# Brown-LEMS/Edge_Based_Visual_Odometry

Hardware: AMD Instinct MI355X
Metric: stereo pairs/sec (TOED+NCC match) on KITTI 1241×376; achieved HBM GB/s (higher is better)
Workload: dtype f64; 1 GPU; configs[1]: single KITTI-shaped stereo pair 1241x376 (generator S2, scene 7+rank, 12 px disparity), TOED both images (fp64, no FMA, bit-exact) + epipolar/disparity/orientation candidate search + NCC, resident in HBM, replayed; toed_mode=hybrid, edges_left=126184, edges_right=126340, candidate_pairs=581657, ncc_matches=472947, sims_stored=False, pairs_in_flight_per_gpu=6, streams_per_gpu=4, pairs_submitted_as_hipgraph=2331, toed_strict_fallbacks=0, parallelism=1 independent sequence(s), one per GPU, no collective

## Files before the change

### edge_based_visual_odometry_amd/csrc/toed_kernels.hip

```cpp
#include <cstring>

#include <hip/hip_ext.h>

#include "ebvo_internal.h"
#include <atomic>
#include "ebvo_math.h"

namespace
{

const double h_TAP_INT[4][19] = {
    {7.99187055345274e-06, 6.69151128824427e-05, 0.000436341347522880, 0.00221592420596900,
     0.00876415024678427, 0.0269954832565940, 0.0647587978329459, 0.120985362259572, 0.176032663382150,
     0.199471140200716, 0.176032663382150, 0.120985362259572, 0.0647587978329459, 0.0269954832565940,
     0.00876415024678427, 0.00221592420596900, 0.000436341347522880, 6.69151128824427e-05,
     7.99187055345274e-06},
    {1.79817087452687e-05, 0.000133830225764885, 0.000763597358165040, 0.00332388630895351,
     0.0109551878084803, 0.0269954832565940, 0.0485690983747094, 0.0604926811297858, 0.0440081658455374, 0,
     -0.0440081658455374, -0.0604926811297858, -0.0485690983747094, -0.0269954832565940,
     -0.0109551878084803, -0.00332388630895351, -0.000763597358165040, -0.000133830225764885,
     -1.79817087452687e-05},
    {3.84608770384913e-05, 0.000250931673309160, 0.00122721003990810, 0.00443184841193801,
     0.0115029471989044, 0.0202466124424455, 0.0202371243227956, 0, -0.0330061243841531,
     -0.0498677850501791, -0.0330061243841531, 0, 0.0202371243227956, 0.0202466124424455,
// ... 569 lines not shown
        {
            const v2f ti0 = *reinterpret_cast<const v2f *>(L.tap[0][0]), ti18 = *reinterpret_cast<const v2f *>(L.tap[0][18]);
            const v2f th0 = *reinterpret_cast<const v2f *>(L.tap[1][0]), th18 = *reinterpret_cast<const v2f *>(L.tap[1][18]);
#pragma unroll
            for (int c = 0; c < 4; ++c)
            {
                const float xl = v[c + HALO + 9], xr = v[c + HALO - 9];
                const v2f l2 = (v2f){xl, xl}, r2 = (v2f){xr, xr};
                const v2f i19 = __builtin_elementwise_fma(r2, ti18, __builtin_elementwise_fma(l2, ti0, a17[c]));
                const v2f h19 = __builtin_elementwise_fma(r2, th18, __builtin_elementwise_fma(l2, th0, ah[c]));
                o[0][c] = a17[c].x;
                o[1][c] = a17[c].y;
                o[2][c] = i19.x;
                o[3][c] = i19.y;
                o[4][c] = h19.x;
                o[5][c] = h19.y;
            }
        }
#pragma unroll
        for (int k = 0; k < 6; ++k)
            *reinterpret_cast<float4 *>(&L.R[k][r][c0]) = make_float4(o[k][0], o[k][1], o[k][2], o[k][3]);
    }
    __syncthreads();
    const int c = tid & 31, ph = (tid >> 5) & 3, sy = ph >> 1, sx = ph & 1, e0 = (tid >> 7) * 7;
    float fx[7], fy[7], mg[7];
    {
        const int base = sx ? 4 : (sy ? 2 : 0);
        const int pm = (ph == 0) ? 8 : 9;
        v2f rr[25];
#pragma unroll
        for (int k = 0; k < 25; ++k)
            rr[k] = (v2f){L.R[base + 1][e0 + k][c], L.R[base][e0 + k][c]};
        v2f acc[7];
#pragma unroll
        for (int e = 0; e < 7; ++e)
            acc[e] = (v2f){0.0f, 0.0f};
#pragma unroll
        for (int p = -9; p <= 9; ++p)
        {
            if (p < -pm || p > pm)
                continue;
            const v2f kk = *reinterpret_cast<const v2f *>(L.tap[sy][p + 9]);
#pragma unroll
            for (int e = 0; e < 7; ++e)
                acc[e] = __builtin_elementwise_fma(rr[e + HALO - p], kk, acc[e]);
        }
#pragma unroll
        for (int e = 0; e < 7; ++e)
        {
            fx[e] = acc[e].x;
            fy[e] = acc[e].y;
        }
        const float dcx = T->screen_dc[ph][0], dcy = T->screen_dc[ph][1];
#pragma unroll
        for (int e = 0; e < 7; ++e)
        {
            fx[e] += dcx;
            fy[e] += dcy;
            mg[e] = __builtin_sqrtf(__builtin_fmaf(fx[e], fx[e], fy[e] * fy[e]));
        }
    }
    __syncthreads();
#pragma unroll
    for (int e = 0; e < 7; ++e)
        L.M[ph][e0 + e][c] = mg[e];
    __syncthreads();
    const float *Mflat = &L.M[0][0][0];
    auto row_step = [&](int da) { return ((((sy + da) & 1) - sy) * 2 * FE_H + ((sy + da) >> 1)) * FE_W; };
    auto col_step = [&](int db) { return (((sx + db) & 1) - sx) * FE_H * FE_W + ((sx + db) >> 1); };
    const int rdn = row_step(-1), rup = row_step(1), cdn = col_step(-1), cup = col_step(1);
    const int lane = tid & 63;
#pragma unroll
    for (int e = 0; e < 7; ++e)
    {
        const int er = e0 + e;
        const int i = i0 + er, j = j0 + c;
        const int I = 2 * i + sy, J = 2 * j + sx;
        int f = 0;
        const bool mine = er >= 1 && er <= FT_H && c >= 1 && c <= FT_W && I >= 10 && I < H2 - 10 && J >= 10 && J < W2 - 10;
        if (mine)
        {
            const float m = mg[e];
            if (m > 2.0f - SCREEN_TOL_M)
            {
                const float gx = fx[e], gy = fy[e], ax = fabsf(gx), ay = fabsf(gy);
                if (ax < SCREEN_TOL_M || ay < SCREEN_TOL_M || fabsf(ax - ay) < SCREEN_TOL_M)
                {
                    const bool px = gx >= 0, py = gy >= 0;
                    const int ctr = (ph * FE_H + er) * FE_W + c;
                    const int rP = py ? rup : rdn, rM = py ? rdn : rup, cP = px ? cup : cdn, cM = px ? cdn : cup;
                    float np, nm, dp, dm, w_up;
                    if (ay < SCREEN_TOL_M || ax < SCREEN_TOL_M)
                    {
                        const bool xd = ay < SCREEN_TOL_M;
                        const int aP = xd ? cP : rP, aM = xd ? cM : rM, o1 = xd ? rup : cup, o2 = xd ? rdn : cdn;
                        np = Mflat[ctr + aP];
                        nm = Mflat[ctr + aM];
                        dp = fmaxf(fabsf(Mflat[ctr + aP + o1] - np), fabsf(Mflat[ctr + aP + o2] - np));
                        dm = fmaxf(fabsf(Mflat[ctr + aM + o1] - nm), fabsf(Mflat[ctr + aM + o2] - nm));
                        w_up = 2.0f * SCREEN_TOL_M / (xd ? ax : ay);
                    }
                    else
                    {
                        np = Mflat[ctr + rP + cP];
                        nm = Mflat[ctr + rM + cM];
                        dp = fmaxf(fabsf(Mflat[ctr + cP] - np), fabsf(Mflat[ctr + rP] - np));
                        dm = fmaxf(fabsf(Mflat[ctr + cM] - nm), fabsf(Mflat[ctr + rM] - nm));
                        w_up = 2.0f * SCREEN_TOL_M / fmaxf(ax, ay);
                    }
                    if (m >= np - (SCREEN_TOL_M + w_up * dp) && m >= nm - (SCREEN_TOL_M + w_up * dm))
                        f = 1;
                }
                else
                {
                    const bool px = gx >= 0, py = gy >= 0;
                    const bool xdom = px ? (py ? gx >= gy : !(gx < ay)) : (py ? !(ax < gy) : ax >= ay);
                    const float num = xdom ? ((px == py) ? gy : -gy) : ((px == py) ? gx : -gx);
                    const float den = xdom ? gx : gy;
                    const float slope = num / den;
                    const int ctr = (ph * FE_H + er) * FE_W + c;
                    const int rP = py ? rup : rdn, rM = py ? rdn : rup, cP = px ? cup : cdn, cM = px ? cdn : cup;
                    const float p1 = Mflat[ctr + (xdom ? cP : rP)], p2 = Mflat[ctr + rP + cP];
                    const float m1 = Mflat[ctr + (xdom ? cM : rM)], m2 = Mflat[ctr + rM + cM];
                    const float fp = p1 * (1 - slope) + p2 * slope;
                    const float fm = m1 * (1 - slope) + m2 * slope;
                    const float tp = SCREEN_TOL_M + SCREEN_TOL_S * fabsf(p2 - p1);
                    const float tm = SCREEN_TOL_M + SCREEN_TOL_S * fabsf(m2 - m1);
                    if (m >= fm - tm && m >= fp - tp)
                        f = 1;
                }
            }
            B.flag[blockIdx.z][(size_t)I * W2 + J] = (uint8_t)f;
            if (DIAG)
            {
                float *dp = D.plane[blockIdx.z];
                const size_t plane = (size_t)H2 * W2, o = (size_t)I * W2 + J;
                dp[o] = fx[e];
                dp[plane + o] = fy[e];
                dp[2 * plane + o] = mg[e];
            }
        }
        const unsigned long long any = __ballot(f != 0);
        if (lane == 0 && any)
        {
            const int ne = __popcll(any & 0xffffffffull), no = __popcll(any >> 32);
            if (ne)
                atomicAdd(&B.row_cnt[blockIdx.z][I], ne);
            if (no)
                atomicAdd(&B.row_cnt[blockIdx.z][H2 + I], no);
        }
    }
}

__global__ __launch_bounds__(256) void toed_compact_phase_kernel(ImgBatch B, int h, int w, int cap)
{
    const int W2 = 2 * w, H2 = 2 * h;
    const int i = 10 + blockIdx.x;
    if (i >= H2 - 10)
        return;
    const uint8_t *flag = B.flag[blockIdx.y] + (size_t)i * W2;
    const int32_t *cnt = B.row_cnt[blockIdx.y];
    int32_t *src = B.src[blockIdx.y];
    int32_t *lists = B.lists[blockIdx.y];
    __shared__ int w_all[4], w_par[2][4], s_sum[4][4];
    const int lane = threadIdx.x & 63, wid = threadIdx.x >> 6;
    auto sum_rows = [&](int r_end, int out[4]) {
        int a[4] = {0, 0, 0, 0};
        for (int r = threadIdx.x; r < r_end; r += 256)
        {
            a[(r & 1) * 2 + 0] += cnt[r];
            a[(r & 1) * 2 + 1] += cnt[H2 + r];
        }
#pragma unroll
        for (int k = 0; k < 4; ++k)
            for (int d = 32; d > 0; d >>= 1)
                a[k] += __shfl_down(a[k], d);
        __syncthreads();
        if (lane == 0)
#pragma unroll
            for (int k = 0; k < 4; ++k)
                s_sum[wid][k] = a[k];
        __syncthreads();
#pragma unroll
        for (int k = 0; k < 4; ++k)
            out[k] = s_sum[0][k] + s_sum[1][k] + s_sum[2][k] + s_sum[3][k];
    };
    int pre[4];
    sum_rows(i, pre);
    if (blockIdx.x == 0)
    {
        int tot[4];
        sum_rows(H2, tot);
        if (threadIdx.x == 0)
        {
            const int all = tot[0] + tot[1] + tot[2] + tot[3];
            const bool over = all > cap;
            int32_t *counts = B.counts[blockIdx.y], *lcount = B.lcount[blockIdx.y];
            counts[2] = over ? 0 : all;
            counts[3] = 0;
            counts[4] = all;
            for (int ph = 0; ph < 4; ++ph)
                lcount[ph] = over ? 0 : tot[ph];
            for (int k = 4; k < 12; ++k)
                lcount[k] = 0;
        }
    }
    int base_all = pre[0] + pre[1] + pre[2] + pre[3];
    int base_ph[2] = {pre[(i & 1) * 2], pre[(i & 1) * 2 + 1]};
    const int par = threadIdx.x & 1;
    const unsigned long long pmask = par ? 0xaaaaaaaaaaaaaaaaull : 0x5555555555555555ull;
    for (int j0 = 10; j0 < W2 - 10; j0 += 256)
    {
        const int j = j0 + threadIdx.x;
        const int f = (j < W2 - 10) ? flag[j] : 0;
        const unsigned long long m_all = __ballot(f != 0);
        const unsigned long long below = (1ull << lane) - 1ull;
        if (lane == 0)
        {
            w_all[wid] = __popcll(m_all);
            w_par[0][wid] = __popcll(m_all & 0x5555555555555555ull);
            w_par[1][wid] = __popcll(m_all & 0xaaaaaaaaaaaaaaaaull);
        }
        __syncthreads();
        int pre_all = 0, tot_all = 0, pre_ph = 0, tot_ph[2] = {0, 0};
#pragma unroll
        for (int k = 0; k < 4; ++k)
        {
            if (k < wid)
            {
                pre_all += w_all[k];
                pre_ph += w_par[par][k];
            }
            tot_all += w_all[k];
            tot_ph[0] += w_par[0][k];
            tot_ph[1] += w_par[1][k];
        }
        if (f)
        {
            const int r_all = base_all + pre_all + __popcll(m_all & below);
            if (r_all < cap)
            {
                src[2 * r_all] = i * W2 + j;
                src[2 * r_all + 1] = -1;
                const int ph = ((i & 1) << 1) | par;
                lists[(size_t)ph * cap + base_ph[par] + pre_ph + __popcll(m_all & pmask & below)] = r_all;
            }
        }
        base_all += tot_all;
        base_ph[0] += tot_ph[0];
        base_ph[1] += tot_ph[1];
        __syncthreads();
    }
}

struct __attribute__((aligned(64))) CandExact
{
    double gx, gy, m, tox, toy;
    int32_t sector;
    int32_t pad0;
    double pad1[2];
};
static_assert(sizeof(CandExact) == 64, "one cache line per candidate");

__host__ __device__ inline size_t mag_tiles_per_row(int W2) { return (size_t)((W2 + 3) >> 2); }
__host__ __device__ inline size_t mag_map_doubles(int H2, int W2) { return (size_t)((H2 + 1) >> 1) * mag_tiles_per_row(W2) * 8; }
__host__ __device__ inline size_t mag_index(int I, int J, int W2)
{
    return ((size_t)(I >> 1) * mag_tiles_per_row(W2) + (size_t)(J >> 2)) * 8 + (size_t)(((I & 1) << 2) | (J & 3));
}

struct ExactBatch
{
    const uint8_t *img[MAX_BATCH];
    const int32_t *src[MAX_BATCH];
    const int32_t *counts[MAX_BATCH];
    int32_t *lists[MAX_BATCH];
    int32_t *lcount[MAX_BATCH];
    CandExact *cd[MAX_BATCH];
    CandRec *rec[MAX_BATCH];
    int32_t *cand_flag[MAX_BATCH];
    int2 *chunk_cnt[MAX_BATCH];
    const uint8_t *flag[MAX_BATCH];
    uint32_t *needbits[MAX_BATCH];
    int32_t *need_cnt[MAX_BATCH];
    double *magmap[MAX_BATCH];
};

__device__ inline void block_append(bool put, int value, int32_t *__restrict__ list, int32_t *__restrict__ counter,
                                    int *s_cnt )
{
    const int lane = threadIdx.x & 63, wid = threadIdx.x >> 6;
    const unsigned long long m = __ballot(put);
    if (lane == 0)
        s_cnt[wid] = __popcll(m);
    __syncthreads();
    if (threadIdx.x == 0)
    {
        const int tot = s_cnt[0] + s_cnt[1] + s_cnt[2] + s_cnt[3];
        s_cnt[4] = tot ? atomicAdd(counter, tot) : 0;
    }
    __syncthreads();
    if (put)
    {
        int pre = 0;
        for (int k = 0; k < wid; ++k)
            pre += s_cnt[k];
        list[s_cnt[4] + pre + __popcll(m & ((1ull << lane) - 1ull))] = value;
    }
    __syncthreads();
}

struct Row24
{
    unsigned long long w0, w1, w2;
};

__device__ inline Row24 fetch_row(const uint8_t *__restrict__ img, int h, int w, int ii, int j)
{
    const int ic = min(max(ii, 0), h - 1);
    const uint8_t *p = img + (size_t)ic * w + (j - HALO);
    Row24 r;
    __builtin_memcpy(&r.w0, p, 8);
    __builtin_memcpy(&r.w1, p + 8, 8);
    __builtin_memcpy(&r.w2, p + 16, 8);
    return r;
}

struct ColMask
{
    unsigned m[5];
};
__device__ inline ColMask column_mask(int w, int j)
{
    const int lo = max(0, HALO - j), hi = min(19, w + HALO - j);
    ColMask c;
#pragma unroll
    for (int d = 0; d < 5; ++d)
    {
        const int a = min(max(lo - 4 * d, 0), 4), b = min(max(hi - 4 * d, 0), 4);
        const unsigned upto_b = b >= 4 ? 0xffffffffu : ((1u << (8 * b)) - 1u);
        const unsigned upto_a = a >= 4 ? 0xffffffffu : ((1u << (8 * a)) - 1u);
        c.m[d] = upto_b & ~upto_a;
    }
    return c;
}

__device__ inline void unpack_row(const Row24 &r, int h, int ii, const ColMask &cm, bool fast, int v[19])
{
    unsigned d[5] = {(unsigned)r.w0, (unsigned)(r.w0 >> 32), (unsigned)r.w1, (unsigned)(r.w1 >> 32), (unsigned)r.w2};
    if (!fast)
    {
        const bool rok = ii >= 0 && ii < h;
#pragma unroll
        for (int k = 0; k < 5; ++k)
            d[k] = rok ? (d[k] & cm.m[k]) : 0u;
    }
#pragma unroll
    for (int k = 0; k < 19; ++k)
        v[18 - k] = (int)((d[k >> 2] >> (8 * (k & 3))) & 0xffu);
}

__device__ inline bool window_inside(int h, int w, int i, int j)
{
    return i >= HALO && i + HALO < h && j >= HALO && j + HALO < w;
}

struct ExactTaps
{
    double tap[2][19][4];
    double prod[17][17][2];
};

__device__ inline void load_exact_taps(ExactTaps &L, const ToedTables *__restrict__ T)
{
    for (int t = threadIdx.x; t < 2 * 19 * 4; t += blockDim.x)
    {
        const int half = t / 76, k = (t % 76) / 4, d = t & 3;
        L.tap[half][k][d] = half ? T->tap_half[d][k] : T->tap_int[d][k];
    }
    for (int t = threadIdx.x; t < 17 * 17; t += blockDim.x)
    {
        const int p = t / 17, q = t % 17;
        L.prod[p][q][0] = T->prod_fx[p][q];
        L.prod[p][q][1] = T->prod_fy[p][q];
    }
    __syncthreads();
}

template <int SY, int SX>
__device__ inline void exact9(const uint8_t *__restrict__ img, int h, int w, const ExactTaps &L, int i, int j,
                              double f[9])
{
    constexpr bool IP = (SY == 0 && SX == 0);
    const double(*ck)[4] = L.tap[SX];
    const double(*rk)[4] = L.tap[SY];
#pragma unroll
    for (int r = 0; r < 9; ++r)
        f[r] = 0.0;
    constexpr int PM = IP ? 8 : 9;
    const bool fast = __all(window_inside(h, w, i, j));
    const ColMask cm = column_mask(w, j);
    Row24 nxt = fetch_row(img, h, w, i + PM, j);
#pragma unroll 1
    for (int p = -PM; p <= PM; ++p)
// ... 90 lines not shown
        const unsigned xcc = __builtin_amdgcn_s_getreg(20 | (0 << 6) | (31 << 11));
        unsigned long long *o = g_wave_trace[which] + (size_t)wave * 4;
        o[0] = t0;
        o[1] = __builtin_amdgcn_s_memrealtime();
        o[2] = ((unsigned long long)xcc << 32) | hw;
        o[3] = (unsigned long long)tasks;
    }
}
extern "C" int ebvo_wave_trace_read(int which, unsigned long long *dst, int n_waves)
{
    return (int)hipMemcpyFromSymbol(dst, HIP_SYMBOL(g_wave_trace), (size_t)n_waves * 32, (size_t)which * 8192 * 32,
                                    hipMemcpyDeviceToHost);
}
#define EBVO_TRACE_BEGIN() const unsigned long long trace_t0 = __builtin_amdgcn_s_memrealtime(); int trace_n = 0
#define EBVO_TRACE_TASK() ++trace_n
#define EBVO_TRACE_END(which) wave_trace(which, wave, trace_t0, trace_n)
#else
#define EBVO_TRACE_BEGIN()
#define EBVO_TRACE_TASK()
#define EBVO_TRACE_END(which)
#endif

struct ExactTask
{
    int im, ph, k0, n;
};

__device__ inline bool exact_task(const ExactBatch &E, int n_img, int cap, int list0, int t, ExactTask &o)
{
    int base = 0;
    for (int ph = 0; ph < 4; ++ph)
        for (int im = 0; im < n_img; ++im)
        {
            const int n = min(E.lcount[im][list0 + ph], cap);
            const int c = (n + 63) >> 6;
            if (t < base + c)
            {
                o.im = im;
                o.ph = ph;
                o.k0 = (t - base) << 6;
                o.n = n;
                return true;
            }
            base += c;
        }
    return false;
}

template <int SY, int SX>
__device__ inline void centre_run(const ExactBatch &E, const ExactTaps &L, int h, int w, int cap, int im, int k, int n)
{
    const int W2 = 2 * w, H2 = 2 * h, wpr = (W2 + 31) >> 5;
    constexpr int PH = (SY << 1) | SX;
    const int32_t *__restrict__ list = E.lists[im] + (size_t)PH * cap;
    CandExact *__restrict__ cd = E.cd[im];
    const uint8_t *__restrict__ flag = E.flag[im];
    if (k < n)
    {
        const int t = list[k];
        const int o = E.src[im][2 * t];
        const int I = o / W2, J = o - I * W2;
        double f[9];
        exact9<SY, SX>(E.img[im], h, w, L, I >> 1, J >> 1, f);
        const double gx = f[0], gy = f[1];
        const double m = sqrt(gx * gx + gy * gy);
        NmsSector S;
        int packed = -1;
        if (nms_sector(m, gx, gy, S))
        {
            packed = (S.a1 + 1) | ((S.b1 + 1) << 2) | ((S.a2 + 1) << 4) | ((S.b2 + 1) << 6);
#pragma unroll
            for (int q = 0; q < 4; ++q)
            {
                const int da = (q & 2) ? S.a2 : S.a1, db = (q & 2) ? S.b2 : S.b1;
                const int nI = (q & 1) ? I - da : I + da, nJ = (q & 1) ? J - db : J + db;
                const int no = nI * W2 + nJ;
                const bool is_cand = nI >= 10 && nI < H2 - 10 && nJ >= 10 && nJ < W2 - 10 && flag[no] == 1;
                if (!is_cand)
                    atomicOr(&E.needbits[im][(size_t)nI * wpr + (nJ >> 5)], 1u << (nJ & 31));
            }
        }
        CandExact r;
        r.gx = gx;
        r.gy = gy;
        r.m = m;
        third_order_dir(f, r.tox, r.toy);
        r.sector = packed;
        r.pad0 = 0;
        r.pad1[0] = r.pad1[1] = 0.0;
        cd[t] = r;
        E.magmap[im][mag_index(I, J, W2)] = m;
    }
}

#ifndef EBVO_CENTRE_WPS
#define EBVO_CENTRE_WPS 0
#endif
#if EBVO_CENTRE_WPS > 0
__global__ __launch_bounds__(256, EBVO_CENTRE_WPS) void toed_exact_centre_kernel(ExactBatch E, const ToedTables *__restrict__ T, int h,
#else
__global__ __launch_bounds__(256) void toed_exact_centre_kernel(ExactBatch E, const ToedTables *__restrict__ T, int h,
#endif
                                                                int w, int cap, int n_img)
{
    __shared__ ExactTaps L;
    EBVO_TRACE_BEGIN();
    load_exact_taps(L, T);
    const int lane = threadIdx.x & 63;
    const int wave = __builtin_amdgcn_readfirstlane((int)(blockIdx.x * 4 + (threadIdx.x >> 6)));
    ExactTask q;
    for (int t = wave; exact_task(E, n_img, cap, 0, t, q); t += gridDim.x * 4)
    {
        EBVO_TRACE_TASK();
        switch (q.ph)
        {
        case 0: centre_run<0, 0>(E, L, h, w, cap, q.im, q.k0 + lane, q.n); break;
        case 1: centre_run<0, 1>(E, L, h, w, cap, q.im, q.k0 + lane, q.n); break;
        case 2: centre_run<1, 0>(E, L, h, w, cap, q.im, q.k0 + lane, q.n); break;
        default: centre_run<1, 1>(E, L, h, w, cap, q.im, q.k0 + lane, q.n); break;
        }
    }
    EBVO_TRACE_END(0);
}

__global__ __launch_bounds__(256) void toed_need_count_kernel(ExactBatch E, int h, int w)
{
    const int W2 = 2 * w, H2 = 2 * h, wpr = (W2 + 31) >> 5;
    const int im = blockIdx.y, I = blockIdx.x * 4 + (threadIdx.x >> 6), lane = threadIdx.x & 63;
    if (I >= H2)
        return;
    const uint32_t *__restrict__ row = E.needbits[im] + (size_t)I * wpr;
    int ne = 0, no = 0;
    for (int k = lane; k < wpr; k += 64)
    {
        const uint32_t v = row[k];
        ne += __popc(v & 0x55555555u);
        no += __popc(v & 0xaaaaaaaau);
    }
    for (int d = 32; d > 0; d >>= 1)
    {
        ne += __shfl_down(ne, d);
        no += __shfl_down(no, d);
    }
    if (lane == 0)
    {
        E.need_cnt[im][I] = ne;
        E.need_cnt[im][H2 + I] = no;
    }
}

__global__ __launch_bounds__(256) void toed_need_compact_kernel(ExactBatch E, int h, int w, int cap)
{
    const int W2 = 2 * w, H2 = 2 * h, wpr = (W2 + 31) >> 5;
    const int I = blockIdx.x, im = blockIdx.y;
    const int32_t *__restrict__ cnt = E.need_cnt[im];
    const bool last = I >= H2 - 2;
    const int mine0 = cnt[I], mine1 = cnt[H2 + I];
    if (!last && mine0 + mine1 == 0)
        return;
    const uint32_t *__restrict__ bits = E.needbits[im];
    int32_t *__restrict__ lists = E.lists[im];
    __shared__ int w_par[2][4], s_sum[4][2];
    const int lane = threadIdx.x & 63, wid = threadIdx.x >> 6;
    int a0 = 0, a1 = 0;
    for (int r = (I & 1) + 2 * threadIdx.x; r < I; r += 512)
    {
        a0 += cnt[r];
        a1 += cnt[H2 + r];
    }
    for (int d = 32; d > 0; d >>= 1)
    {
        a0 += __shfl_down(a0, d);
        a1 += __shfl_down(a1, d);
    }
    if (lane == 0)
    {
        s_sum[wid][0] = a0;
        s_sum[wid][1] = a1;
    }
    __syncthreads();
    int base_ph[2] = {s_sum[0][0] + s_sum[1][0] + s_sum[2][0] + s_sum[3][0], s_sum[0][1] + s_sum[1][1] + s_sum[2][1] + s_sum[3][1]};
    if (last && threadIdx.x == 0)
    {
        const int n0 = base_ph[0] + mine0, n1 = base_ph[1] + mine1;
        E.lcount[im][4 + 2 * (I & 1) + 0] = n0;
        E.lcount[im][4 + 2 * (I & 1) + 1] = n1;
        atomicAdd(const_cast<int32_t *>(E.counts[im]) + 3, n0 + n1);
    }
    if (mine0 + mine1 == 0)
        return;
    const int par = threadIdx.x & 1;
    const unsigned long long pmask = par ? 0xaaaaaaaaaaaaaaaaull : 0x5555555555555555ull;
    for (int J0 = 0; J0 < W2; J0 += 256)
    {
        const int J = J0 + threadIdx.x;
        const int o = I * W2 + J;
        const bool f = J < W2 && ((bits[(size_t)I * wpr + (J >> 5)] >> (J & 31)) & 1u);
        const unsigned long long m_all = __ballot(f);
        const unsigned long long below = (1ull << lane) - 1ull;
        if (lane == 0)
        {
            w_par[0][wid] = __popcll(m_all & 0x5555555555555555ull);
            w_par[1][wid] = __popcll(m_all & 0xaaaaaaaaaaaaaaaaull);
        }
        __syncthreads();
        int pre_ph = 0, tot_ph[2] = {0, 0};
#pragma unroll
        for (int k = 0; k < 4; ++k)
        {
            if (k < wid)
                pre_ph += w_par[par][k];
            tot_ph[0] += w_par[0][k];
            tot_ph[1] += w_par[1][k];
        }
        if (f)
        {
            const int ph = ((I & 1) << 1) | par;
            const int pos = base_ph[par] + pre_ph + __popcll(m_all & pmask & below);
            if (pos < cap)
                lists[(size_t)(4 + ph) * cap + pos] = o;
        }
        base_ph[0] += tot_ph[0];
        base_ph[1] += tot_ph[1];
        __syncthreads();
    }
}

template <int SY, int SX>
__device__ inline void mags_run(const ExactBatch &E, const ExactTaps &L, int h, int w, int cap, int im, int k, int n)
{
    const int W2 = 2 * w;
    constexpr int PH = (SY << 1) | SX;
    const int32_t *__restrict__ list = E.lists[im] + (size_t)(4 + PH) * cap;
    if (k < n)
    {
        const int o = list[k];
        const int I = o / W2, J = o - I * W2;
        E.magmap[im][mag_index(I, J, W2)] = exact_mag<SY, SX>(E.img[im], h, w, L, I, J);
    }
}

__global__ __launch_bounds__(256) void toed_exact_mags_kernel(ExactBatch E, const ToedTables *__restrict__ T, int h,
                                                              int w, int cap, int n_img)
{
    __shared__ ExactTaps L;
    EBVO_TRACE_BEGIN();
    load_exact_taps(L, T);
    const int lane = threadIdx.x & 63;
    const int wave = __builtin_amdgcn_readfirstlane((int)(blockIdx.x * 4 + (threadIdx.x >> 6)));
    ExactTask q;
    for (int t = wave; exact_task(E, n_img, cap, 4, t, q); t += gridDim.x * 4)
    {
        EBVO_TRACE_TASK();
        switch (q.ph)
        {
        case 0: mags_run<0, 0>(E, L, h, w, cap, q.im, q.k0 + lane, q.n); break;
        case 1: mags_run<0, 1>(E, L, h, w, cap, q.im, q.k0 + lane, q.n); break;
        case 2: mags_run<1, 0>(E, L, h, w, cap, q.im, q.k0 + lane, q.n); break;
        default: mags_run<1, 1>(E, L, h, w, cap, q.im, q.k0 + lane, q.n); break;
        }
    }
    EBVO_TRACE_END(1);
}

__global__ __launch_bounds__(256) void toed_exact_decide_kernel(ExactBatch E, int h, int w, int cap)
{
    __shared__ int s_cnt[4][2];
    const int im = blockIdx.y, W2 = 2 * w;
    const CandExact *__restrict__ cd = E.cd[im];
    CandRec *__restrict__ rec = E.rec[im];
    int32_t *__restrict__ ft = E.cand_flag[im], *__restrict__ fk = ft + cap;
    const int n = min(E.counts[im][2], cap);
    for (int c = blockIdx.x; c * 256 < n; c += gridDim.x)
    {
        const int t = c * 256 + threadIdx.x;
        bool is_max = false;
        int kept = 0;
        if (t < n)
        {
            const int o = E.src[im][2 * t];
            const int I = o / W2, J = o - I * W2;
            const CandExact ce = cd[t];
            const double gx = ce.gx, gy = ce.gy, m = ce.m;
            NmsSector S;
            double px = 0, py = 0, sm = 0;
            if (ce.sector >= 0 && nms_sector(m, gx, gy, S))
            {
                const double *__restrict__ mm = E.magmap[im];
                is_max = nms_finish(m, S, I, J, mm[mag_index(I + S.a1, J + S.b1, W2)], mm[mag_index(I + S.a2, J + S.b2, W2)],
                                    mm[mag_index(I - S.a1, J - S.b1, W2)], mm[mag_index(I - S.a2, J - S.b2, W2)], px, py, sm);
            }
            CandRec r;
            r.x = r.y = r.smag = 0.0;
            r.tox = ce.tox;
            r.toy = ce.toy;
            if (is_max)
            {
                r.x = (px - 1) / 2;
                r.y = (py - 1) / 2;
                r.smag = sm;
                kept = (r.x > 10 && r.x < w - 10 && r.y > 10 && r.y < h - 10) ? 1 : 0;
            }
            rec[t] = r;
            ft[t] = is_max ? 1 : 0;
            fk[t] = kept;
        }
        const unsigned long long bm = __ballot(is_max), bk = __ballot(kept != 0);
        if ((threadIdx.x & 63) == 0)
        {
            s_cnt[threadIdx.x >> 6][0] = __popcll(bm);
            s_cnt[threadIdx.x >> 6][1] = __popcll(bk);
        }
        __syncthreads();
        if (threadIdx.x == 0)
            E.chunk_cnt[im][c] = make_int2(s_cnt[0][0] + s_cnt[1][0] + s_cnt[2][0] + s_cnt[3][0],
                                           s_cnt[0][1] + s_cnt[1][1] + s_cnt[2][1] + s_cnt[3][1]);
        __syncthreads();
    }
}


__global__ __launch_bounds__(256) void toed_screen_audit_kernel(ExactBatch E, ScreenDiag D, int h, int w, int cap, int im,
                                                                unsigned long long *out)
{
    const int W2 = 2 * w, H2 = 2 * h;
    const size_t plane = (size_t)H2 * W2;
    const float *__restrict__ dp = D.plane[im];
    const int n = min(E.counts[im][2], cap);
    double e[4] = {0, 0, 0, 0};
    for (int t = blockIdx.x * blockDim.x + threadIdx.x; t < n; t += gridDim.x * blockDim.x)
    {
        const int o = E.src[im][2 * t];
        const CandExact ce = E.cd[im][t];
        e[0] = fmax(e[0], fabs((double)dp[o] - ce.gx));
        e[1] = fmax(e[1], fabs((double)dp[plane + o] - ce.gy));
        e[2] = fmax(e[2], fabs((double)dp[2 * plane + o] - ce.m));
    }
    for (int ph = 0; ph < 4; ++ph)
    {
        const int32_t *__restrict__ list = E.lists[im] + (size_t)(4 + ph) * cap;
        const int np = min(E.lcount[im][4 + ph], cap);
        for (int k = blockIdx.x * blockDim.x + threadIdx.x; k < np; k += gridDim.x * blockDim.x)
        {
            const int o = list[k];
            const int I = o / W2, J = o - I * W2;
            if (I >= 10 && I < H2 - 10 && J >= 10 && J < W2 - 10)
                e[3] = fmax(e[3], fabs((double)dp[2 * plane + o] - E.magmap[im][mag_index(I, J, W2)]));
        }
    }
#pragma unroll
    for (int k = 0; k < 4; ++k)
        if (e[k] > 0)
            atomicMax(&out[k], (unsigned long long)__double_as_longlong(e[k]));
    if (blockIdx.x == 0 && threadIdx.x == 0)
        out[5] = (unsigned long long)n;
}

__global__ __launch_bounds__(256) void toed_cand_scatter_kernel(ImgBatch B, int cap)
{
    __shared__ int s_base[4][2], s_in[4][2];
    const CandRec *__restrict__ rec = B.rec[blockIdx.y];
    const int32_t *__restrict__ ftp = B.cand_flag[blockIdx.y], *__restrict__ fkp = ftp + cap;
    const int2 *__restrict__ chunk_cnt = reinterpret_cast<const int2 *>(B.cand_off[blockIdx.y]);
    ebvo_edge *__restrict__ edges = B.edges[blockIdx.y];
    double *__restrict__ all4 = B.all4[blockIdx.y];
    int32_t *counts = B.counts[blockIdx.y];
    const int n = min(counts[2], cap);
    const int lane = threadIdx.x & 63, wid = threadIdx.x >> 6;
    if (n == 0 && blockIdx.x == 0 && threadIdx.x == 0)
    {
        counts[0] = 0;
        counts[1] = 0;
    }
    for (int c = blockIdx.x; c * 256 < n; c += gridDim.x)
    {
        int a0 = 0, a1 = 0;
        for (int k = threadIdx.x; k < c; k += 256)
// ... 65 lines not shown
    }
}

}

int toed_init_constants(ebvo_ctx *ctx)
{
    static ToedTables host;
    memcpy(host.tap_int, h_TAP_INT, sizeof(h_TAP_INT));
    memcpy(host.tap_half, h_TAP_HALF, sizeof(h_TAP_HALF));
    for (int p = -8; p <= 8; ++p)
        for (int q = -8; q <= 8; ++q)
        {
            host.prod_fx[p + 8][q + 8] = h_TAP_INT[1][q + 9] * h_TAP_INT[0][p + 9];
            host.prod_fy[p + 8][q + 8] = h_TAP_INT[0][q + 9] * h_TAP_INT[1][p + 9];
        }
    for (int sy = 0; sy < 2; ++sy)
        for (int sx = 0; sx < 2; ++sx)
        {
            const int pm = (sy == 0 && sx == 0) ? 8 : 9;
            const double(*xt)[19] = sx ? h_TAP_HALF : h_TAP_INT, (*yt)[19] = sy ? h_TAP_HALF : h_TAP_INT;
            double sxg = 0, sxgx = 0, syg = 0, sygx = 0;
            for (int q = -pm; q <= pm; ++q)
            {
                sxg += xt[0][q + 9];
                sxgx += xt[1][q + 9];
                syg += yt[0][q + 9];
                sygx += yt[1][q + 9];
            }
            host.screen_dc[(sy << 1) | sx][0] = (float)(127.5 * sxgx * syg);
            host.screen_dc[(sy << 1) | sx][1] = (float)(127.5 * sxg * sygx);
        }
    if (ctx->device < 0 || ctx->device >= 16)
        return EBVO_ERR_ARG;
    if (!g_tables_dev[ctx->device])
    {
        ToedTables *d = nullptr;
        EBVO_HIP(ctx, hipMalloc(&d, sizeof(ToedTables)));
        EBVO_HIP(ctx, hipMemcpy(d, &host, sizeof(ToedTables), hipMemcpyHostToDevice));
        g_tables_dev[ctx->device] = d;
    }
    return EBVO_OK;
}

static int resident_blocks(ebvo_ctx *ctx, int which)
{
    if (ctx->exact_blocks[which] > 0)
        return ctx->exact_blocks[which];
    static std::atomic<int> cached[16][2];
    std::atomic<int> &slot = cached[ctx->device & 15][which];
    int c = slot.load(std::memory_order_relaxed);
    if (c == 0)
    {
        int per_cu = 0, cus = 0;
        if (which == 0)
            (void)hipOccupancyMaxActiveBlocksPerMultiprocessor(&per_cu, toed_exact_centre_kernel, 256, 0);
        else
            (void)hipOccupancyMaxActiveBlocksPerMultiprocessor(&per_cu, toed_exact_mags_kernel, 256, 0);
        (void)hipDeviceGetAttribute(&cus, hipDeviceAttributeMultiprocessorCount, ctx->device);
        c = (per_cu > 0 ? per_cu : 4) * (cus > 0 ? cus : 256);
        slot.store(c, std::memory_order_relaxed);
    }
    return c;
}

unsigned long long *toed_screen_audit_result(Slot &s, int k, int h, int w)
{
    const int H2 = 2 * h, W2 = 2 * w;
    const int need_words = H2 * ((W2 + 31) / 32);
    float *planes = (float *)((int32_t *)(s.im[k].maps + mag_map_doubles(H2, W2)) + need_words + 4 * H2);
    return (unsigned long long *)(planes + 3 * (size_t)H2 * W2);
}

void toed_screen_budget(double out[5])
{
    out[0] = SCREEN_E_G;
    out[1] = SCREEN_E_M;
    out[2] = SCREEN_E_S;
    out[3] = SCREEN_TOL_M;
    out[4] = SCREEN_TOL_S;
}

int toed_enqueue(ebvo_ctx *ctx, Slot &s, int n_img, int h, int w, hipEvent_t ev_conv_begin, hipEvent_t ev_conv_end,
                 hipEvent_t ev_end, int mode, bool want_all4)
{
    if (n_img < 1 || n_img > MAX_BATCH)
        return EBVO_ERR_ARG;
    if (mode < 0)
        mode = ctx->toed_mode;
    const int H2 = 2 * h, W2 = 2 * w;
    const int need_words = H2 * ((W2 + 31) / 32);
    ImgBatch B{};
    for (int k = 0; k < n_img; ++k)
    {
        ImageWS &ws = s.im[k];
        B.img[k] = ws.img;
        B.maps[k] = ws.maps;
        B.flag[k] = ws.flag;
        B.row_cnt[k] = ws.row_cnt;
        B.row_off[k] = ws.row_off;
        B.counts[k] = ws.counts;
        B.src[k] = ws.src;
        B.edges[k] = ws.edges;
        B.all4[k] = want_all4 ? ws.all4 : nullptr;
        B.rec[k] = (CandRec *)ws.cand_rec;
        B.cand_flag[k] = ws.cand_flag;
        B.cand_off[k] = ws.cand_off;
        B.lists[k] = ws.cand_lists;
        B.lcount[k] = ws.cand_lcount;
    }
    {
        int32_t *ptrs[2 * MAX_BATCH];
        int counts[2 * MAX_BATCH];
        int nc = 0;
        for (int k = 0; k < n_img; ++k)
        {
            ptrs[nc] = s.im[k].row_cnt;
            counts[nc++] = 2 * H2;
            if (mode == EBVO_TOED_HYBRID)
            {
                ptrs[nc] = (int32_t *)(s.im[k].maps + mag_map_doubles(H2, W2));
                counts[nc++] = need_words;
            }
        }
        int rc = ebvo_clear_enqueue(ctx, s, ptrs, counts, nc);
        if (rc)
            return rc;
    }
    if (mode == EBVO_TOED_HYBRID)
    {
        const int cap = ctx->cap_edges;
        ScreenDiag D{};
        if (ev_conv_begin)
            EBVO_HIP(ctx, hipEventRecord(ev_conv_begin, s.stream));
        {
            ProfScope ps(ctx, s, K_NMS);
            const dim3 ftiles((w + FT_W - 1) / FT_W, (h + FT_H - 1) / FT_H, n_img);
            if (ctx->screen_audit)
            {
                for (int k = 0; k < n_img; ++k)
                    D.plane[k] = (float *)((int32_t *)(s.im[k].maps + mag_map_doubles(H2, W2)) + need_words + 4 * H2);
                hipLaunchKernelGGL(toed_screen_fused_kernel<true>, ftiles, dim3(256), 0, s.stream, B,
                                   (const ToedTables *)g_tables_dev[ctx->device], h, w, D);
            }
            else
                hipLaunchKernelGGL(toed_screen_fused_kernel<false>, ftiles, dim3(256), 0, s.stream, B,
                                   (const ToedTables *)g_tables_dev[ctx->device], h, w, D);
        }
        const int stop = ctx->stop_stage;
        if (stop == 1)
            return EBVO_OK;
        {
            ProfScope ps(ctx, s, K_COMPACT);
            hipLaunchKernelGGL(toed_compact_phase_kernel, dim3(H2 - 20, n_img), dim3(256), 0, s.stream, B, h, w, cap);
        }
        if (stop == 2)
            return EBVO_OK;
        {
            ExactBatch E{};
            for (int k = 0; k < n_img; ++k)
            {
                ImageWS &ws = s.im[k];
                E.img[k] = ws.img;
                E.src[k] = ws.src;
                E.counts[k] = ws.counts;
                E.lists[k] = ws.cand_lists;
                E.lcount[k] = ws.cand_lcount;
                E.cd[k] = (CandExact *)ws.cand_data;
                E.rec[k] = (CandRec *)ws.cand_rec;
                E.cand_flag[k] = ws.cand_flag;
                E.chunk_cnt[k] = reinterpret_cast<int2 *>(ws.cand_off);
                E.flag[k] = ws.flag;
                E.magmap[k] = ws.maps;
                E.needbits[k] = (uint32_t *)(ws.maps + mag_map_doubles(H2, W2));
                E.need_cnt[k] = (int32_t *)(E.needbits[k] + need_words);
            }
            const ToedTables *T = (const ToedTables *)g_tables_dev[ctx->device];
            {
                hipEvent_t k_begin, k_end;
                if (ebvo_prof_kernel(ctx, s, K_EXACT_CENTRE, &k_begin, &k_end))
                    hipExtLaunchKernelGGL(toed_exact_centre_kernel, dim3(resident_blocks(ctx, 0)), dim3(256), 0, s.stream,
                                          k_begin, k_end, 0, E, T, h, w, cap, n_img);
                else
                    hipLaunchKernelGGL(toed_exact_centre_kernel, dim3(resident_blocks(ctx, 0)), dim3(256), 0, s.stream, E,
                                       T, h, w, cap, n_img);
                if (ctx->repeat_mask & 1)
                    hipLaunchKernelGGL(toed_exact_centre_kernel, dim3(resident_blocks(ctx, 0)), dim3(256), 0, s.stream, E,
                                       T, h, w, cap, n_img);
            }
            if (stop == 3)
                return EBVO_OK;
            {
                ProfScope ps(ctx, s, K_COMPACT);
                hipLaunchKernelGGL(toed_need_count_kernel, dim3((H2 + 3) / 4, n_img), dim3(256), 0, s.stream, E, h, w);
                hipLaunchKernelGGL(toed_need_compact_kernel, dim3(H2, n_img), dim3(256), 0, s.stream, E, h, w, cap);
            }
            if (stop == 4)
                return EBVO_OK;
            {
                ProfScope ps(ctx, s, K_EXACT_MAGS);
                hipLaunchKernelGGL(toed_exact_mags_kernel, dim3(resident_blocks(ctx, 1)), dim3(256), 0, s.stream, E, T, h,
                                   w, cap, n_img);
                if (ctx->repeat_mask & 2)
                    hipLaunchKernelGGL(toed_exact_mags_kernel, dim3(resident_blocks(ctx, 1)), dim3(256), 0, s.stream, E, T, h,
                                       w, cap, n_img);
                if (stop == 5)
                    return EBVO_OK;
                hipLaunchKernelGGL(toed_exact_decide_kernel, dim3(512 / (ctx->small_div > 0 ? ctx->small_div : 4), n_img), dim3(256), 0, s.stream, E, h, w, cap);
            }
            if (stop == 6)
                return EBVO_OK;
            if (ctx->screen_audit)
                for (int k = 0; k < n_img; ++k)
                {
                    unsigned long long *out = toed_screen_audit_result(s, k, h, w);
                    EBVO_HIP(ctx, hipMemsetAsync(out, 0, 8 * sizeof(unsigned long long), s.stream));
                    hipLaunchKernelGGL(toed_screen_audit_kernel, dim3(512), dim3(256), 0, s.stream, E, D, h, w, cap, k, out);
                }
        }
        if (ev_conv_end)
            EBVO_HIP(ctx, hipEventRecord(ev_conv_end, s.stream));
        {
            ProfScope ps(ctx, s, K_FINALIZE);
            hipLaunchKernelGGL(toed_cand_scatter_kernel, dim3(512 / (ctx->small_div > 0 ? ctx->small_div : 4), n_img), dim3(256), 0, s.stream, B, cap);
        }
        if (ev_end)
            EBVO_HIP(ctx, hipEventRecord(ev_end, s.stream));
        EBVO_HIP(ctx, hipGetLastError());
        return EBVO_OK;
    }
    if (ev_conv_begin)
        EBVO_HIP(ctx, hipEventRecord(ev_conv_begin, s.stream));
    {
        ProfScope ps(ctx, s, K_CONV);
        dim3 grid((w + TILE_W - 1) / TILE_W, (h + TILE_H - 1) / TILE_H, 2 * n_img);
        hipLaunchKernelGGL(toed_conv_kernel, grid, dim3(256), 0, s.stream, B,
                           (const ToedTables *)g_tables_dev[ctx->device], h, w);
    }
    if (ev_conv_end)
        EBVO_HIP(ctx, hipEventRecord(ev_conv_end, s.stream));
    {
        ProfScope ps(ctx, s, K_NMS);
        dim3 grid((W2 - 20 + 63) / 64, (H2 - 20 + 3) / 4, n_img);
        hipLaunchKernelGGL(toed_nms_kernel, grid, dim3(64, 4), 0, s.stream, B, h, w);
    }
    {
        ProfScope ps(ctx, s, K_ROWSCAN);
        hipLaunchKernelGGL(toed_rowscan_kernel, dim3(n_img), dim3(64), 0, s.stream, B, H2, 0);
    }
    {
        ProfScope ps(ctx, s, K_COMPACT);
        hipLaunchKernelGGL(toed_compact_kernel, dim3(H2 - 20, n_img), dim3(256), 0, s.stream, B, h, w, ctx->cap_edges);
    }
    {
        ProfScope ps(ctx, s, K_FINALIZE);
        hipLaunchKernelGGL(toed_finalize_kernel, dim3(512, n_img), dim3(256), 0, s.stream, B, h, w, ctx->cap_edges);
    }
    if (ev_end)
        EBVO_HIP(ctx, hipEventRecord(ev_end, s.stream));
    EBVO_HIP(ctx, hipGetLastError());
    return EBVO_OK;
}
```

Before: 3535 stereo pairs/s.

## Compact rows one-per-wave with DPP scans and packed flag bitmasks

Both row-compaction kernels now assign one row per wavefront instead of one row per 256-thread block, so they no longer need shared memory or __syncthreads. Each lane reads 8 flag bytes (or a 32-bit need word) and turns them into a bitmask. A DPP-based wave exclusive scan packs the even and odd phase counts into the two 16-bit halves of one integer, and set bits are walked serially per lane. This is meant to cut barrier and ballot overhead and per-block launch cost, at the risk of divergent serial bit-walks and unaligned 8-byte loads. The launch grids are divided by four to match.

Measured after the change: 3598 stereo pairs/s (median of 6 runs). 1.02x the previous value.

```diff
diff --git a/edge_based_visual_odometry_amd/csrc/toed_kernels.hip b/edge_based_visual_odometry_amd/csrc/toed_kernels.hip
--- a/edge_based_visual_odometry_amd/csrc/toed_kernels.hip
+++ b/edge_based_visual_odometry_amd/csrc/toed_kernels.hip
@@ -745,46 +745,87 @@
     }
 }
 
+template <int CTRL>
+__device__ inline int dpp_i32(int v)
+{
+    return __builtin_amdgcn_update_dpp(0, v, CTRL, 0xf, 0xf, true);
+}
+
+__device__ inline void wave_sum4(int a[4])
+{
+#pragma unroll
+    for (int k = 0; k < 4; ++k)
+    {
+        int v = a[k];
+        v += dpp_i32<0xB1>(v);
+        v += dpp_i32<0x4E>(v);
+        v += dpp_i32<0x141>(v);
+        v += dpp_i32<0x140>(v);
+        a[k] = __builtin_amdgcn_readlane(v, 0) + __builtin_amdgcn_readlane(v, 16) + __builtin_amdgcn_readlane(v, 32) +
+               __builtin_amdgcn_readlane(v, 48);
+    }
+}
+
+__device__ inline unsigned wave_excl_scan_pair(unsigned x, unsigned &total)
+{
+    int v = (int)x;
+    v += dpp_i32<0x111>(v);
+    v += dpp_i32<0x112>(v);
+    v += dpp_i32<0x114>(v);
+    v += dpp_i32<0x118>(v);
+    const int t0 = __builtin_amdgcn_readlane(v, 15), t1 = __builtin_amdgcn_readlane(v, 31),
+              t2 = __builtin_amdgcn_readlane(v, 47), t3 = __builtin_amdgcn_readlane(v, 63);
+    const int row = (int)(threadIdx.x & 63) >> 4;
+    const int front = (row > 0 ? t0 : 0) + (row > 1 ? t1 : 0) + (row > 2 ? t2 : 0);
+    total = (unsigned)(t0 + t1 + t2 + t3);
+    return (unsigned)(v + front) - x;
+}
+
+template <class Emit>
+__device__ inline void walk_set_bits(unsigned m, Emit emit)
+{
+    while (__any(m != 0u))
+    {
+        if (m)
+        {
+            const int b = __ffs((int)m) - 1;
+            m &= m - 1u;
+            emit(b);
+        }
+    }
+}
+
 __global__ __launch_bounds__(256) void toed_compact_phase_kernel(ImgBatch B, int h, int w, int cap)
 {
     const int W2 = 2 * w, H2 = 2 * h;
-    const int i = 10 + blockIdx.x;
+    const int lane = threadIdx.x & 63;
+    const int i = __builtin_amdgcn_readfirstlane(10 + (int)blockIdx.x * 4 + (int)(threadIdx.x >> 6));
     if (i >= H2 - 10)
         return;
-    const uint8_t *flag = B.flag[blockIdx.y] + (size_t)i * W2;
+    const uint8_t *flag = B.flag[blockIdx.y] + (size_t)i * W2 + 10;
     const int32_t *cnt = B.row_cnt[blockIdx.y];
     int32_t *src = B.src[blockIdx.y];
     int32_t *lists = B.lists[blockIdx.y];
-    __shared__ int w_all[4], w_par[2][4], s_sum[4][4];
-    const int lane = threadIdx.x & 63, wid = threadIdx.x >> 6;
     auto sum_rows = [&](int r_end, int out[4]) {
-        int a[4] = {0, 0, 0, 0};
-        for (int r = threadIdx.x; r < r_end; r += 256)
-        {
-            a[(r & 1) * 2 + 0] += cnt[r];
-            a[(r & 1) * 2 + 1] += cnt[H2 + r];
-        }
-#pragma unroll
-        for (int k = 0; k < 4; ++k)
-            for (int d = 32; d > 0; d >>= 1)
-                a[k] += __shfl_down(a[k], d);
-        __syncthreads();
-        if (lane == 0)
-#pragma unroll
-            for (int k = 0; k < 4; ++k)
-                s_sum[wid][k] = a[k];
-        __syncthreads();
-#pragma unroll
-        for (int k = 0; k < 4; ++k)
-            out[k] = s_sum[0][k] + s_sum[1][k] + s_sum[2][k] + s_sum[3][k];
+        int se = 0, so = 0;
+        for (int r = lane; r < r_end; r += 64)
+        {
+            se += cnt[r];
+            so += cnt[H2 + r];
+        }
+        out[0] = lane & 1 ? 0 : se;
+        out[1] = lane & 1 ? 0 : so;
+        out[2] = lane & 1 ? se : 0;
+        out[3] = lane & 1 ? so : 0;
+        wave_sum4(out);
     };
     int pre[4];
     sum_rows(i, pre);
-    if (blockIdx.x == 0)
+    if (i == 10)
     {
         int tot[4];
         sum_rows(H2, tot);
-        if (threadIdx.x == 0)
+        if (lane == 0)
         {
             const int all = tot[0] + tot[1] + tot[2] + tot[3];
             const bool over = all > cap;
@@ -799,50 +840,44 @@
         }
     }
     int base_all = pre[0] + pre[1] + pre[2] + pre[3];
-    int base_ph[2] = {pre[(i & 1) * 2], pre[(i & 1) * 2 + 1]};
-    const int par = threadIdx.x & 1;
-    const unsigned long long pmask = par ? 0xaaaaaaaaaaaaaaaaull : 0x5555555555555555ull;
-    for (int j0 = 10; j0 < W2 - 10; j0 += 256)
-    {
-        const int j = j0 + threadIdx.x;
-        const int f = (j < W2 - 10) ? flag[j] : 0;
-        const unsigned long long m_all = __ballot(f != 0);
-        const unsigned long long below = (1ull << lane) - 1ull;
-        if (lane == 0)
-        {
-            w_all[wid] = __popcll(m_all);
-            w_par[0][wid] = __popcll(m_all & 0x5555555555555555ull);
-            w_par[1][wid] = __popcll(m_all & 0xaaaaaaaaaaaaaaaaull);
-        }
-        __syncthreads();
-        int pre_all = 0, tot_all = 0, pre_ph = 0, tot_ph[2] = {0, 0};
-#pragma unroll
-        for (int k = 0; k < 4; ++k)
-        {
-            if (k < wid)
-            {
-                pre_all += w_all[k];
-                pre_ph += w_par[par][k];
-            }
-            tot_all += w_all[k];
-            tot_ph[0] += w_par[0][k];
-            tot_ph[1] += w_par[1][k];
-        }
-        if (f)
-        {
-            const int r_all = base_all + pre_all + __popcll(m_all & below);
+    int base_e = pre[(i & 1) * 2], base_o = pre[(i & 1) * 2 + 1];
+    int32_t *list_e = lists + (size_t)((i & 1) << 1) * cap;
+    const int ncol = W2 - 20;
+    for (int c0 = 0; c0 < ncol; c0 += 512)
+    {
+        const int c = c0 + 8 * lane;
+        unsigned mask = 0;
+        if (c < ncol)
+        {
+            unsigned long long x;
+            __builtin_memcpy(&x, flag + c, 8);
+            const unsigned lo = (unsigned)x, hi = (unsigned)(x >> 32);
+            const unsigned tl = ((((lo & 0x7f7f7f7fu) + 0x7f7f7f7fu) | lo) >> 7) & 0x01010101u;
+            const unsigned th = ((((hi & 0x7f7f7f7fu) + 0x7f7f7f7fu) | hi) >> 7) & 0x01010101u;
+            mask = ((tl * 0x01020408u) >> 24) | (((th * 0x01020408u) >> 24) << 4);
+            if (ncol - c < 8)
+                mask &= (1u << (ncol - c)) - 1u;
+        }
+        unsigned total;
+        const unsigned front = wave_excl_scan_pair((unsigned)__popc(mask & 0x55u) | ((unsigned)__popc(mask & 0xaau) << 16), total);
+        int r_all = base_all + (int)(front & 0xffffu) + (int)(front >> 16);
+        int p_e = base_e + (int)(front & 0xffffu), p_o = base_o + (int)(front >> 16);
+        const int o0 = i * W2 + 10 + c;
+        walk_set_bits(mask, [&](int b) {
+            const int par = b & 1;
             if (r_all < cap)
             {
-                src[2 * r_all] = i * W2 + j;
+                src[2 * r_all] = o0 + b;
                 src[2 * r_all + 1] = -1;
-                const int ph = ((i & 1) << 1) | par;
-                lists[(size_t)ph * cap + base_ph[par] + pre_ph + __popcll(m_all & pmask & below)] = r_all;
-            }
-        }
-        base_all += tot_all;
-        base_ph[0] += tot_ph[0];
-        base_ph[1] += tot_ph[1];
-        __syncthreads();
+                list_e[(par ? p_o : p_e) + (cap & -par)] = r_all;
+            }
+            ++r_all;
+            p_o += par;
+            p_e += par ^ 1;
+        });
+        base_all += (int)(total & 0xffffu) + (int)(total >> 16);
+        base_e += (int)(total & 0xffffu);
+        base_o += (int)(total >> 16);
     }
 }
 
@@ -1239,77 +1274,53 @@
 __global__ __launch_bounds__(256) void toed_need_compact_kernel(ExactBatch E, int h, int w, int cap)
 {
     const int W2 = 2 * w, H2 = 2 * h, wpr = (W2 + 31) >> 5;
-    const int I = blockIdx.x, im = blockIdx.y;
+    const int im = blockIdx.y, lane = threadIdx.x & 63;
+    const int I = __builtin_amdgcn_readfirstlane((int)blockIdx.x * 4 + (int)(threadIdx.x >> 6));
+    if (I >= H2)
+        return;
     const int32_t *__restrict__ cnt = E.need_cnt[im];
     const bool last = I >= H2 - 2;
     const int mine0 = cnt[I], mine1 = cnt[H2 + I];
     if (!last && mine0 + mine1 == 0)
         return;
-    const uint32_t *__restrict__ bits = E.needbits[im];
-    int32_t *__restrict__ lists = E.lists[im];
-    __shared__ int w_par[2][4], s_sum[4][2];
-    const int lane = threadIdx.x & 63, wid = threadIdx.x >> 6;
-    int a0 = 0, a1 = 0;
-    for (int r = (I & 1) + 2 * threadIdx.x; r < I; r += 512)
-    {
-        a0 += cnt[r];
-        a1 += cnt[H2 + r];
-    }
-    for (int d = 32; d > 0; d >>= 1)
-    {
-        a0 += __shfl_down(a0, d);
-        a1 += __shfl_down(a1, d);
-    }
-    if (lane == 0)
-    {
-        s_sum[wid][0] = a0;
-        s_sum[wid][1] = a1;
-    }
-    __syncthreads();
-    int base_ph[2] = {s_sum[0][0] + s_sum[1][0] + s_sum[2][0] + s_sum[3][0], s_sum[0][1] + s_sum[1][1] + s_sum[2][1] + s_sum[3][1]};
-    if (last && threadIdx.x == 0)
-    {
-        const int n0 = base_ph[0] + mine0, n1 = base_ph[1] + mine1;
+    const uint32_t *__restrict__ bits = E.needbits[im] + (size_t)I * wpr;
+    int a[4] = {0, 0, 0, 0};
+    for (int r = (I & 1) + 2 * lane; r < I; r += 128)
+    {
+        a[0] += cnt[r];
+        a[1] += cnt[H2 + r];
+    }
+    wave_sum4(a);
+    int base_e = a[0], base_o = a[1];
+    if (last && lane == 0)
+    {
+        const int n0 = base_e + mine0, n1 = base_o + mine1;
         E.lcount[im][4 + 2 * (I & 1) + 0] = n0;
         E.lcount[im][4 + 2 * (I & 1) + 1] = n1;
         atomicAdd(const_cast<int32_t *>(E.counts[im]) + 3, n0 + n1);
     }
     if (mine0 + mine1 == 0)
         return;
-    const int par = threadIdx.x & 1;
-    const unsigned long long pmask = par ? 0xaaaaaaaaaaaaaaaaull : 0x5555555555555555ull;
-    for (int J0 = 0; J0 < W2; J0 += 256)
-    {
-        const int J = J0 + threadIdx.x;
-        const int o = I * W2 + J;
-        const bool f = J < W2 && ((bits[(size_t)I * wpr + (J >> 5)] >> (J & 31)) & 1u);
-        const unsigned long long m_all = __ballot(f);
-        const unsigned long long below = (1ull << lane) - 1ull;
-        if (lane == 0)
-        {
-            w_par[0][wid] = __popcll(m_all & 0x5555555555555555ull);
-            w_par[1][wid] = __popcll(m_all & 0xaaaaaaaaaaaaaaaaull);
-        }
-        __syncthreads();
-        int pre_ph = 0, tot_ph[2] = {0, 0};
-#pragma unroll
-        for (int k = 0; k < 4; ++k)
-        {
-            if (k < wid)
-                pre_ph += w_par[par][k];
-            tot_ph[0] += w_par[0][k];
-            tot_ph[1] += w_par[1][k];
-        }
-        if (f)
-        {
-            const int ph = ((I & 1) << 1) | par;
-            const int pos = base_ph[par] + pre_ph + __popcll(m_all & pmask & below);
+    int32_t *__restrict__ list_e = E.lists[im] + (size_t)(4 + ((I & 1) << 1)) * cap;
+    for (int k0 = 0; k0 < wpr; k0 += 64)
+    {
+        const int k = k0 + lane;
+        unsigned v = k < wpr ? bits[k] : 0u;
+        if (W2 - 32 * k < 32)
+            v &= W2 - 32 * k > 0 ? (1u << (W2 - 32 * k)) - 1u : 0u;
+        unsigned total;
+        const unsigned front = wave_excl_scan_pair((unsigned)__popc(v & 0x55555555u) | ((unsigned)__popc(v & 0xaaaaaaaau) << 16), total);
+        int p_e = base_e + (int)(front & 0xffffu), p_o = base_o + (int)(front >> 16);
+        const int o0 = I * W2 + 32 * k;
+        walk_set_bits(v, [&](int b) {
+            const int par = b & 1, pos = par ? p_o : p_e;
             if (pos < cap)
-                lists[(size_t)(4 + ph) * cap + pos] = o;
-        }
-        base_ph[0] += tot_ph[0];
-        base_ph[1] += tot_ph[1];
-        __syncthreads();
+                list_e[pos + (cap & -par)] = o0 + b;
+            p_o += par;
+            p_e += par ^ 1;
+        });
+        base_e += (int)(total & 0xffffu);
+        base_o += (int)(total >> 16);
     }
 }
 
@@ -1681,7 +1692,7 @@
             return EBVO_OK;
         {
             ProfScope ps(ctx, s, K_COMPACT);
-            hipLaunchKernelGGL(toed_compact_phase_kernel, dim3(H2 - 20, n_img), dim3(256), 0, s.stream, B, h, w, cap);
+            hipLaunchKernelGGL(toed_compact_phase_kernel, dim3((H2 - 20 + 3) / 4, n_img), dim3(256), 0, s.stream, B, h, w, cap);
         }
         if (stop == 2)
             return EBVO_OK;
@@ -1722,7 +1733,7 @@
             {
                 ProfScope ps(ctx, s, K_COMPACT);
                 hipLaunchKernelGGL(toed_need_count_kernel, dim3((H2 + 3) / 4, n_img), dim3(256), 0, s.stream, E, h, w);
-                hipLaunchKernelGGL(toed_need_compact_kernel, dim3(H2, n_img), dim3(256), 0, s.stream, E, h, w, cap);
+                hipLaunchKernelGGL(toed_need_compact_kernel, dim3((H2 + 3) / 4, n_img), dim3(256), 0, s.stream, E, h, w, cap);
             }
             if (stop == 4)
                 return EBVO_OK;
```
